# Nature40/pyradiotracking

Measured on AMD Instinct MI355X. Metric: IQ MSamples/s analysed (STFT + detect + records), detected-signal parity vs CPU, higher is better.
Workload: dtype f32

## Files before the change

### pyradiotracking_amd/csrc/rt_analyze.hip

```cpp
#include <hip/hip_runtime.h>

#include <algorithm>
#include <cmath>
#include <cstdio>
#include <cstdlib>
#include <cstring>
#include <limits>
#include <new>
#include <string>
#include <type_traits>
#include <vector>

#include "rt_kernels.h"
#include "rt_general.h"
#include "rt_f64.h"
#include "rt_f64_sparse.h"
#include "rt_f64_rescue.h"
#include "rt_cells.h"
#include "rt_present.h"
#include "rt_chain.h"
#include "rt_record_iq.h"
#include "rt_record_stft.h"
#include "rt_record_stft_hop.h"
#include "rt_record_band.h"
// ... 770 lines not shown
        if (!gone && marked) rows[(size_t)kMaskSubList * S + n_sub++] = s;
        if (!gone && !marked) rows[(size_t)kMaskLinList * S + n_lin++] = s;
    }
    *n_lin_present = n_lin;
    *n_sub_present = n_sub;
    *n_absent = n_abs;
}

int upload_mask(rt_handle *h, Slot &sl) {
    const int S = h->cfg.n_streams;
    fill_mask_rows(sl.lc.pc, S, h->lin ? h->h_sub_first.data() : nullptr, sl.h_mask, &sl.n_lin_present, &sl.n_sub_present, &sl.n_absent);
    RT_HIP(h, hipMemcpyAsync(sl.d_mask, sl.h_mask, (size_t)kMaskRows * S * sizeof(int32_t), hipMemcpyHostToDevice, h->s_scan));
    return RT_OK;
}

int upload_chain_rows(rt_handle *h, Slot &sl) {
    const size_t S = (size_t)h->cfg.n_streams;
    std::memcpy(sl.h_chain_rows, sl.lc.cc.src_buf.data(), S * sizeof(int32_t));
    std::memcpy(sl.h_chain_rows + S, sl.lc.cc.src_idx.data(), S * sizeof(int32_t));
    RT_HIP(h, hipMemcpyAsync(sl.d_chain_rows, sl.h_chain_rows, 2 * S * sizeof(int32_t), hipMemcpyHostToDevice, h->s_scan));
    return RT_OK;
}

template <class P>
int enqueue_carry(rt_handle *h, const int32_t *d_absent_list, int n_absent, const P *src, P *dst, int K, int N) {
    const int64_t per = (int64_t)K * N;
    if (n_absent == 0 || per <= 0) return RT_OK;
    const int bps = carry_blocks(per);
    hipLaunchKernelGGL((carry_tails<P>), dim3((unsigned)((int64_t)n_absent * bps)), dim3(kCarryBlock), 0, h->s_scan, d_absent_list, n_absent, bps, src, dst, per);
    RT_HIP(h, hipGetLastError());
    return RT_OK;
}

int enqueue_analysis(rt_handle *h, Slot &sl, int mode, bool *launched = nullptr, bool second_pass_only = false, bool own_means = false) {
    sl.call.rec_cap_used = h->rec_cap;
    const CallCtx &c = sl.call;
    if (mode == RT_MODE_RUNFILTER && c.thr_rerun && !second_pass_only) own_means = true;
    if (launched) *launched = false;
    const MaskedLaunches masked_launches(h, sl);
    const int32_t *const absent = sl.lc.masked ? sl.d_mask + (size_t)kMaskAbsent * h->cfg.n_streams : nullptr;
    if (h->general) {
        int rc = ensure_dense_spec(h);
        if (rc != RT_OK) return rc;
        RT_HIP(h, hipEventRecord(sl.ev_begin, h->s_scan));
        if (launched) *launched = true;
        launch_general(h, c.iq, c.stream_stride, c.n_seg, h->d_spec, h->d_tail[c.tail_write], c.fmt, absent);
        {
            const int64_t cells = (int64_t)h->cfg.n_streams * h->N;
            hipLaunchKernelGGL(row_sums_dense, dim3((unsigned)((cells + 255) / 256)), dim3(256), 0, h->s_scan, h->d_spec, sl.d_psum, h->cfg.n_streams, c.n_seg, h->N);
        }
        RT_HIP(h, hipGetLastError());
        { const int rc2 = enqueue_chain(h, sl, h->s_scan); if (rc2 != RT_OK) return rc2; }
        RT_HIP(h, hipEventRecord(sl.ev_scan, h->s_scan));
        DetectArgs a = make_detect_args(h, sl, c.n_seg, h->N, c.n_seg_last);
        a.prev = call_prev(h, sl);
        a.prev_cols = h->K;
        a.spec = h->d_spec;
        a.psum = sl.d_psum;
        a.chunks = 1;
        launch_detect_dense(h, h->cfg.n_streams, h->s_scan, a);
        RT_HIP(h, hipGetLastError());
        { const int rc2 = enqueue_row_means(h, sl, 1, c.n_seg, h->s_scan); if (rc2 != RT_OK) return rc2; }
        { const int rc2 = enqueue_record_cells(h, sl, h->d_spec, nullptr, 0, h->s_scan); if (rc2 != RT_OK) return rc2; }
        RT_HIP(h, hipEventRecord(sl.ev_done, h->s_scan));
        return RT_OK;
    }
// ... 139 lines not shown
            const double span = (double)(t_max - t_min);
            std::fprintf(stderr, "RT_STAMPS launch span %.1f us, %.2f waves resident per SIMD on average, %.1f %% of a wave's life inside the step loop; ",
                         span / 100.0, resident / span / 1024.0, 100.0 * sum[13] / resident);
            const double steps = sum[11];
            double tot = 0;
            for (int k = 0; k <= 10; ++k) tot += sum[k];
            std::fprintf(stderr, "RT_STAMPS nperseg %d: %.0f waves, %.1f steps per wave, %.0f cycles per step, in-kernel clock %.0f MHz:", h->N, waves,
                         steps / waves, tot / steps, sum[13] > 0 ? sum[12] / sum[13] * 100.0 : 0.0);
            for (int k = 0; k <= 10; ++k) std::fprintf(stderr, " [%d] %.0f", k, sum[k] / steps);
            std::fprintf(stderr, "\n");
        }
#endif
    }
    RT_HIP(h, hipGetLastError());
    const bool two_scans = !dense && (mode == RT_MODE_RUNFILTER || mode == RT_MODE_PREFILTER);
    { const int rc = enqueue_chain(h, sl, two_scans ? s2 : h->s_scan); if (rc != RT_OK) return rc; }
    RT_HIP(h, hipEventRecord(sl.ev_scan, two_scans ? s2 : h->s_scan));
    if (sd != (two_scans ? s2 : h->s_scan)) RT_HIP(h, hipStreamWaitEvent(sd, sl.ev_scan, 0));
    DetectArgs a = make_detect_args(h, sl, c.n_seg, h->N, c.n_seg_last);
    a.prev = call_prev(h, sl);
    a.prev_cols = h->K;
    a.chunks = sp.blocks_per_stream;
    a.spec = h->d_spec;
    a.filtered = (mode == RT_MODE_PREFILTER || mode == RT_MODE_RUNFILTER) ? 1 : 0;
    if (mode == RT_MODE_RUNFILTER) {
        a.seg_total = sp.seg_count + S;
        a.host_seg_total = sl.h_seg_total;
    }
    if (dense) {
        launch_detect_dense(h, S, sd, a);
    } else {
        if (a.work_list) {
            hipLaunchKernelGGL(detect_group, dim3((S + 3) / 4), dim3(256), h->lds_small, sd, a);
            hipLaunchKernelGGL(detect_bucket_listed, dim3(std::min(S * kQuarters, 1024)), dim3(256), h->lds_small, sd, a);
        } else {
            const int waves = S * kBuckets;
            hipLaunchKernelGGL(detect_bucket<false>, dim3((waves + 3) / 4), dim3(256), h->lds_small, sd, a);
        }
        hipLaunchKernelGGL(detect_bucket<true>, dim3(S), dim3(256), h->lds_large, sd, a);
        if (sl.d_cells) hipLaunchKernelGGL(cells_keep_counts, dim3((S * kBuckets + 255) / 256), dim3(256), 0, sd, sl.d_hot_count, sl.d_hot_kept, S * kBuckets);
        hipLaunchKernelGGL(finalize_records, dim3(S), dim3(256), 0, sd, a);
    }
    RT_HIP(h, hipGetLastError());
    { const int rc = enqueue_row_means(h, sl, sp.blocks_per_stream, c.n_seg, sd); if (rc != RT_OK) return rc; }
    { const int rc = enqueue_record_cells(h, sl, dense ? h->d_spec : nullptr, nullptr, 0, sd); if (rc != RT_OK) return rc; }
    RT_HIP(h, hipEventRecord(sl.ev_done, sd));
    return RT_OK;
}

int enqueue_partial_dense(rt_handle *h, Slot &sl, int n_list, unsigned long long records_so_far) {
    const CallCtx &c = sl.call;
    const int n_part = std::min(h->cfg.n_streams, kMaxPartial);
    if (!h->d_spec_part) {
        const size_t bytes = (size_t)n_part * (size_t)h->max_seg * (size_t)h->N * sizeof(float);
        hipError_t e = hipMalloc(&h->d_spec_part, bytes ? bytes : 4);
        if (e != hipSuccess) {
            h->d_spec_part = nullptr;
            h->err = "dense spectrogram scratch for the partial re-run (" + std::to_string(bytes) + " bytes): " + hipGetErrorString(e);
            return RT_E_NOMEM;
        }
    }
    StftParams sp = make_stft_params(h, sl, c.iq, c.stream_stride, c.n_seg, c.tail_write);
    sp.n_streams = n_list;
    sp.stream_list = sl.h_list;
    sp.spec = h->d_spec_part;
    *sl.h_total = records_so_far;
    RT_HIP(h, hipMemcpyAsync(sl.d_counters, sl.h_total, sizeof(unsigned long long), hipMemcpyHostToDevice, h->s_scan));
    launch_scan<1>(h, sp, n_list * sp.blocks_per_stream, c.fmt);
    RT_HIP(h, hipGetLastError());
    { const int rc = enqueue_chain(h, sl, h->s_scan); if (rc != RT_OK) return rc; }
    DetectArgs a = make_detect_args(h, sl, c.n_seg, h->N, c.n_seg_last);
    a.prev = call_prev(h, sl);
// ... 1567 lines not shown
        if (cfg->mode == RT_MODE_PREFILTER && !h->ap.lv.prefilter_ok) {
            delete h;
            return fail_create(RT_E_UNSUPPORTED, "RT_MODE_PREFILTER needs signal_min_duration >= 2 * segs_per_chunk STFT hops");
        }
        h->two_level = scan_wave64(R3) && !h->ap.lv.prefilter_ok && !RT_DIAG_ENV("RT_EXP_ONE_LEVEL");
        if (h->two_level) {
            h->max_chunks += h->max_chunks / 4 + 2;
            max_blocks_per_stream = (h->max_chunks + h->GPW - 1) / h->GPW;
            h->max_blocks = max_blocks_per_stream;
        }
        h->run_cells = (int)std::max<long long>(1, std::min<long long>(r_min, 1 << 20));
        const bool fits = !general && !big && h->LG >= 4 && std::min<long long>(h->run_cells, (long long)h->max_seg + 1) <= kPlanMaxRun && h->max_seg >= 2;
        if (cfg->mode == RT_MODE_RUNFILTER && !fits) {
            delete h;
            return fail_create(RT_E_UNSUPPORTED, "RT_MODE_RUNFILTER: the minimum plateau length (in STFT hops) is beyond the planner's counters");
        }
        h->ap.lv.runfilter_ok = fits && (cfg->mode == RT_MODE_RUNFILTER || cfg->mode == RT_MODE_AUTO);
        if (h->ap.lv.runfilter_ok && cfg->mode == RT_MODE_AUTO) {
            const size_t per_slot = (size_t)cfg->n_streams * std::max(h->max_seg, 1) * (size_t)(h->LG * 4 + 4) + (size_t)cfg->n_streams * h->N * 4 * (size_t)(h->max_blocks + 2);
            size_t free_b = 0, total_b = 0;
            if (hipMemGetInfo(&free_b, &total_b) != hipSuccess || (size_t)kSlots * per_slot > free_b / (h->ap.lv.prefilter_ok ? 8 : 2)) h->ap.lv.runfilter_ok = false;
        }
    }
    if (!general && ((long long)h->N << key_tbits(std::max(h->max_seg, 2))) > 0x100000000ll) {
        delete h;
        return fail_create(RT_E_UNSUPPORTED, "max_samples too large for 32-bit cell keys");
    }
    h->hot_cap = general ? 64
                 : cfg->hot_capacity > 0
                     ? cfg->hot_capacity
                     : std::min(8192, std::max(kSmallBucket, next_pow2(std::max(h->max_seg, 1)) * std::max(1, h->N / 1024)));
    h->lds_dense = rec_lds_bytes(h->rec_cap);
    {
        h->cand_cap = (h->N / kBuckets <= 32) ? 32 : kCandCapMax;
        const size_t tail = (((size_t)(h->N / kBuckets) * 4 + 15) & ~(size_t)15) + sizeof(rt_record) * h->cand_cap;
        h->lds_large = (size_t)next_pow2(std::max(h->hot_cap, 64)) * 8 + tail;
        h->lds_small = 4 * ((size_t)kSmallBucket * 8 + tail);
    }
    if (h->lds_large + 8 * 1024 > 160 * 1024) {
        delete h;
        return fail_create(RT_E_INVALID, "hot_capacity does not fit the 160 KiB LDS of a CU");
    }
    {
        int fbits = 0;
        while ((1 << fbits) < h->N) ++fbits;
        const bool can = !general && h->N <= kGroupBins && fbits + key_tbits(std::max(h->max_seg, 1)) + 10 <= 32;
        const bool want = (cfg->flags & RT_FLAG_GROUP_DETECT) ? true : (cfg->flags & RT_FLAG_NO_GROUP_DETECT) ? false
                          : cfg->n_streams >= 1024 || (g_creating_lane && (cfg->flags & kFlagLaneOfLargeBatch));
        h->group_detect = can && want;
        h->group_forced = (cfg->flags & RT_FLAG_GROUP_DETECT) != 0;
    }

    auto fail = [&](int code, const std::string &msg) {
        std::string m = msg;
        rt_destroy(h);
        return fail_create(code, m);
    };
#define RT_CREATE_HIP(expr)                                                                  \
    do {                                                                                     \
        hipError_t e2_ = (expr);                                                             \
        if (e2_ != hipSuccess) return fail(RT_E_HIP, std::string(#expr) + ": " + hipGetErrorString(e2_)); \
    } while (0)

    if (cfg->hip_stream) {
        h->s_scan = static_cast<hipStream_t>(cfg->hip_stream);
        h->s_detect = h->s_scan;
    } else {
        RT_CREATE_HIP(hipStreamCreateWithFlags(&h->s_scan, hipStreamNonBlocking));
        h->own_scan_stream = true;
        bool second = R3 <= 2 && !big && !g_creating_lane;
// ... 117 lines not shown
        RT_CREATE_HIP(hipHostMalloc(&sl.h_dc_flag, (size_t)S * sizeof(int32_t)));
        std::memset(sl.h_dc_flag, 0, (size_t)S * sizeof(int32_t));
        RT_CREATE_HIP(hipHostMalloc(&sl.h_list, (size_t)kMaxPartial * sizeof(int32_t)));
        RT_CREATE_HIP(hipHostMalloc(&sl.h_total, sizeof(unsigned long long)));
        if (cfg->flags & RT_FLAG_ROW_MEANS) RT_CREATE_HIP(hipMalloc(&sl.d_row_means, (size_t)S * N * sizeof(float)));
        if (cfg->flags & RT_FLAG_RECORD_CELLS) {
            sl.cell_cap = std::max<int64_t>(64, std::min<int64_t>(kInitialPoolCells, 16 * sl.pool_cap));
            RT_CREATE_HIP(hipMalloc(&sl.d_cells, (size_t)sl.cell_cap * sizeof(float)));
            RT_DEVICE_ZEROS(RT_CREATE_HIP, sl.d_hot_kept, (size_t)S * kBuckets * sizeof(uint32_t));
            RT_CREATE_HIP(hipMalloc(&sl.d_stream_cells, (size_t)S * sizeof(long long)));
            RT_CREATE_HIP(hipMalloc(&sl.d_stream_base, (size_t)S * sizeof(long long)));
            RT_CREATE_HIP(hipHostMalloc(&sl.h_cells_info, 2 * sizeof(unsigned long long)));
            sl.h_cells_info[0] = sl.h_cells_info[1] = 0ull;
        }
        RT_CREATE_HIP(hipEventCreate(&sl.ev_begin));
        RT_CREATE_HIP(hipEventCreateWithFlags(&sl.ev_first, hipEventDisableTiming));
        RT_CREATE_HIP(hipEventCreate(&sl.ev_scan));
        RT_CREATE_HIP(hipEventCreate(&sl.ev_done));
    }

    if (big) {
#define RT_WG_SET(B_, M_, U_, W_) RT_CREATE_HIP(hipFuncSetAttribute(reinterpret_cast<const void *>(stft_wg<B_, M_, U_, W_>), hipFuncAttributeMaxDynamicSharedMemorySize, (int)wg_lds_bytes(B_)))
#define RT_WG_SET4(B_, M_) RT_WG_SET(B_, M_, false, false); RT_WG_SET(B_, M_, false, true); RT_WG_SET(B_, M_, true, false); RT_WG_SET(B_, M_, true, true); \
    RT_WG_SET(B_, M_ | kModeI16, false, false); RT_WG_SET(B_, M_ | kModeI16, false, true); \
    RT_WG_SET(B_, M_ | kModeI8, false, false); RT_WG_SET(B_, M_ | kModeI8, false, true)
        RT_WG_SET4(256, 0); RT_WG_SET4(256, 1); RT_WG_SET4(256, 2);
        RT_WG_SET4(512, 0); RT_WG_SET4(512, 1); RT_WG_SET4(512, 2);
#undef RT_WG_SET4
#undef RT_WG_SET
    }
    RT_CREATE_HIP(hipFuncSetAttribute(reinterpret_cast<const void *>(detect_bucket<true>),
                                      hipFuncAttributeMaxDynamicSharedMemorySize, (int)h->lds_large));
    RT_CREATE_HIP(hipFuncSetAttribute(reinterpret_cast<const void *>(detect_bucket<false>),
                                      hipFuncAttributeMaxDynamicSharedMemorySize, (int)h->lds_small));
    RT_CREATE_HIP(hipFuncSetAttribute(reinterpret_cast<const void *>(detect_group), hipFuncAttributeMaxDynamicSharedMemorySize, (int)h->lds_small));
    RT_CREATE_HIP(hipFuncSetAttribute(reinterpret_cast<const void *>(detect_bucket_listed), hipFuncAttributeMaxDynamicSharedMemorySize, (int)h->lds_small));
    RT_CREATE_HIP(hipFuncSetAttribute(reinterpret_cast<const void *>(detect_dense<false>), hipFuncAttributeMaxDynamicSharedMemorySize,
                                      (int)rec_lds_bytes(kDenseLdsRecords)));
#undef RT_CREATE_HIP
    *out = h;
    return RT_OK;
}

int rt_reset(rt_handle *h) {
    if (!h) return RT_E_INVALID;
    forget_row_means(h);
    for (rt_handle *k : h->kids) rt_reset(k);
    h->ledger.forget_all();
    return RT_OK;
}

int rt_reset_stream(rt_handle *h, int32_t stream) {
    if (!h) return RT_E_INVALID;
    if (stream < 0 || stream >= h->cfg.n_streams) {
        h->err = "stream index out of range";
        return RT_E_INVALID;
    }
    if (!h->kids.empty()) {
        for (size_t k = 0; k < h->kids.size(); ++k)
            if (stream < h->kid_base[k + 1]) return rt_reset_stream(h->kids[k], stream - h->kid_base[k]);
        return RT_E_INVALID;
    }
    h->ledger.reset_stream(stream);
    return RT_OK;
}

static int refuse_on_f64(rt_handle *h, const char *what, const char *twin) {
    h->err = std::string(what) + " on a float64 handle (rt_create_f64): " + (twin ? std::string("use ") + twin : std::string("not available"));
    return RT_E_INVALID;
// ... 2038 lines not shown
```

### pyradiotracking_amd/csrc/rt_core.h

```cpp
#ifndef RT_CORE_H
#define RT_CORE_H

#include <math.h>
#include <stdint.h>

#include <algorithm>
#include <cmath>
#include <initializer_list>
#include <type_traits>
#include <utility>
#include <vector>

#if defined(__HIP__)
#define RT_HD __host__ __device__ __forceinline__
#else
#define RT_HD inline
#endif

namespace rt {

struct cf {
    float x, y;
};
struct cd {
// ... 163 lines not shown


inline int tail_cols(int nperseg, double fs, double max_d) {
    const double hop = seg_time(1, nperseg, fs) - seg_time(0, nperseg, fs);
    const double k = std::floor(max_d / hop) + 2.0;
    const int K = (int)std::min(k, 1.0e6);
    return K < 1 ? 1 : K;
}

inline long long min_run_cells(int N, double fs, double min_d) {
    const double hop = seg_time(1, N, fs) - seg_time(0, N, fs);
    const double cells = min_d * (1.0 - 1e-9) / hop;
    return (long long)std::ceil(std::min(cells, 1.0e9)) - 1;
}

inline int next_pow2(int v) {
    int p = 1;
    while (p < v) p <<= 1;
    return p;
}

inline int key_tbits(int n_seg) {
    int t = 1;
    while ((1ll << t) < (long long)n_seg) ++t;
    return t;
}

constexpr int kBuckets = 16;
constexpr int kSmallBucket = 1024;
constexpr int kQuarters = 4;
constexpr int kCandCapMax = 64;
constexpr int kGroupCells = 896;
constexpr int kGroupBins = 256;

constexpr int kGeneralMaxN = 16384;
struct ScanFamily {
    int R3 = 0, QS = 0, big = 0;
    bool general = false, bluestein = false;
    bool supported = false;
};
inline ScanFamily scan_family(int nperseg) {
    ScanFamily f;
    for (int r : {1, 2, 4, 8, 16})
        if (nperseg == 256 * r) f.R3 = r;
    for (int q : {2, 4, 8})
        if (nperseg == 16 * q) {
            f.R3 = 1;
            f.QS = q;
        }
    if (nperseg == 8192 || nperseg == 16384) {
        f.R3 = 1;
        f.big = nperseg / 32;
    }
    f.supported = true;
    if (!f.R3) {
        const int n = nperseg;
        const bool pow2 = n > 0 && (n & (n - 1)) == 0;
        f.supported = !(n < 8 || (pow2 && n > kGeneralMaxN) || (!pow2 && n > kGeneralMaxN / 2));
        f.general = true;
        f.bluestein = !pow2;
        f.R3 = 1;
    }
    return f;
}

inline int choose_chunk(int nperseg, int R3, int QS, int block, double fs, double min_duration_s, int segs_per_chunk, int n_streams, int n_seg) {
// ... 515 lines not shown
```

### pyradiotracking_amd/csrc/rt_hostcheck.cpp

```cpp
#include <algorithm>
#include <cstdint>
#include <cstring>
#include <numeric>
#include <vector>

#include "../../include/rt_analyze.h"
#include "rt_core.h"
#include "rt_input_stats.h"
#include "rt_ledger.h"
#include "rt_record_stft_book.h"
#include "rt_tables.h"

using namespace rt;

extern "C" {

long long hc_timedelta_us(double seconds) { return (long long)timedelta_us(seconds); }

int hc_probe_stride(int nperseg, double fs, double min_d) { return probe_stride(nperseg, fs, min_d); }

double hc_seg_time(int k, int nperseg, double fs) { return seg_time(k, nperseg, fs); }

int hc_tail_cols(int nperseg, double fs, double max_d) { return tail_cols(nperseg, fs, max_d); }

// ... 193 lines not shown
    return total;
}
}

extern "C" {
long long hc_record_cells(const float *spec, int n_bins, const float *last, int n_seg_last, const rt_record *rec, int n, long long *offsets,
                          float *cells, long long cap) {
    return record_cells_host(spec, n_bins, last, n_seg_last, rec, n, offsets, cells, cap);
}
long long hc_record_cells_f64(const double *spec, int n_bins, const double *last, int n_seg_last, const rt_record_f64 *rec, int n,
                              long long *offsets, double *cells, long long cap) {
    return record_cells_host(spec, n_bins, last, n_seg_last, rec, n, offsets, cells, cap);
}
}

extern "C" {

void hc_scan_family(int nperseg, int *out) {
    const ScanFamily f = scan_family(nperseg);
    const int v[6] = {f.R3, f.QS, f.big, f.general, f.bluestein, f.supported};
    std::memcpy(out, v, sizeof v);
}
int hc_choose_chunk(int nperseg, int block, double fs, double min_d, int segs_per_chunk, int n_streams, int n_seg) {
    const ScanFamily f = scan_family(nperseg);
    return choose_chunk(nperseg, f.R3, f.QS, block, fs, min_d, segs_per_chunk, n_streams, n_seg);
}
long long hc_min_run_cells(int nperseg, double fs, double min_d) { return min_run_cells(nperseg, fs, min_d); }
int hc_key_tbits(int n_seg) { return key_tbits(n_seg); }
void hc_detect_order_constants(int *out) {
    const int v[6] = {kBuckets, kSmallBucket, kGroupCells, kGroupBins, kQuarters, kCandCapMax};
    std::memcpy(out, v, sizeof v);
}
int hc_next_pow2(int v) { return next_pow2(v); }

void hc_scan_twiddles(int N, int R3, int QS, int big, int wave64, cf *tw1, cf *tw2, int *n) {
    const ScanTwiddles t = scan_twiddles(N, R3, QS, big, wave64 != 0);
    n[0] = (int)t.tw1.size();
    n[1] = (int)t.tw2.size();
    if (tw1) std::memcpy(tw1, t.tw1.data(), t.tw1.size() * sizeof(cf));
    if (tw2) std::memcpy(tw2, t.tw2.data(), t.tw2.size() * sizeof(cf));
}
void hc_scaled_window(const float *window, int N, float scale, float *ws) {
    const std::vector<float> v = scaled_window(window, N, scale);
    std::memcpy(ws, v.data(), v.size() * sizeof(float));
}
void hc_window_thread_order(const float *ws, int N, int big, float *out) {
    const std::vector<float> v = window_thread_order(std::vector<float>(ws, ws + N), N, big);
    std::memcpy(out, v.data(), v.size() * sizeof(float));
}
void hc_window_lane_order(const float *ws, int N, int LG, int wave64, float *out) {
    const std::vector<float> v = window_lane_order(std::vector<float>(ws, ws + N), N, LG, wave64 != 0);
    std::memcpy(out, v.data(), v.size() * sizeof(float));
}
int hc_fit_cosine_window(const float *ws, int N, double *wr, double *wi) {
    const CosineFit f = fit_cosine_window(std::vector<float>(ws, ws + N), N);
    std::memcpy(wr, f.wr, sizeof f.wr);
    std::memcpy(wi, f.wi, sizeof f.wi);
    return f.cosine_sum ? 1 : 0;
}
void hc_transform_twiddles_f32(int M, cf *out) {
    const std::vector<cf> v = transform_twiddles<cf, double>(M);
    std::memcpy(out, v.data(), v.size() * sizeof(cf));
}
void hc_transform_twiddles_f64(int M, cd *out) {
    const std::vector<cd> v = transform_twiddles<cd, long double>(M);
    std::memcpy(out, v.data(), v.size() * sizeof(cd));
// ... 481 lines not shown
```

### pyradiotracking_amd/csrc/rt_kernels.h

```cpp
#ifndef RT_KERNELS_H
#define RT_KERNELS_H

#include <hip/hip_runtime.h>
#include <stdint.h>

#include <type_traits>

#include "../../include/rt_analyze.h"
#include "rt_diag.h"
#include "rt_core.h"
#include "rt_fft.h"

namespace rt {

constexpr int kBlock = 256;
constexpr int kRowF2 = 18;

struct StftParams {
    const void *iq;
    int64_t stream_stride;
    int32_t n_streams;
    int32_t n_seg;
    int32_t segs_per_chunk;
    int32_t chunks;
// ... 397 lines not shown
            const u4 v = __builtin_nontemporal_load(reinterpret_cast<const u4 *>(p + 4 * h));
            dst[(4 * h) * QS + m] = iq_i16{v.x};
            dst[(4 * h + 1) * QS + m] = iq_i16{v.y};
            dst[(4 * h + 2) * QS + m] = iq_i16{v.z};
            dst[(4 * h + 3) * QS + m] = iq_i16{v.w};
        }
    }
}

#ifndef RT_ONE_WAVE_MAX_R3
#define RT_ONE_WAVE_MAX_R3 0
#endif
#ifndef RT_NO_PERSIST
#define RT_NO_PERSIST 0
#endif
__device__ __forceinline__ int g_of(unsigned tid, int lg) { return (int)tid / lg; }
__host__ __device__ constexpr bool scan_persistent(int R3, int mode) { return mode != 5 && mode != 7 && !RT_NO_PERSIST && R3 >= 4; }
__host__ __device__ constexpr int scan_block(int R3) { return R3 <= RT_ONE_WAVE_MAX_R3 ? 64 : kBlock; }

#ifndef RT_EXP_DMA1024
#define RT_EXP_DMA1024 0
#endif
constexpr int kModeI16 = 16, kModeI8 = 32;
__host__ __device__ constexpr int scan_fmt(int modef, bool u8) { return (modef & kModeI8) ? kFmtI8 : (modef & kModeI16) ? kFmtI16 : u8 ? kFmtU8 : kFmtC64; }
__host__ __device__ constexpr bool scan_dma(int r3, int fmt, int qs) { return RT_EXP_DMA1024 && r3 == 4 && fmt == kFmtC64 && qs == 0; }
__device__ void raw_buffer_load_lds_fwd(rsrc_t rsrc, __attribute__((address_space(3))) void *lds, int size, int voffset, int soffset, int offset, int aux)
    __asm("llvm.amdgcn.raw.buffer.load.lds");
#ifndef RT_WG4_MAX_R3
#define RT_WG4_MAX_R3 0
#endif
#ifndef RT_PK_R3_MASK
#define RT_PK_R3_MASK (1 | 4)
#endif
#ifndef RT_EXP_U8_PK
#define RT_EXP_U8_PK 0
#endif
__host__ __device__ constexpr int scan_wgs_per_cu(int r3, int fmt, int qs) {
    return scan_dma(r3, fmt, qs) ? 2 : (r3 <= RT_WG4_MAX_R3 || (fmt == kFmtU8 && r3 == 1 && !RT_EXP_U8_PK)) ? 4 : 3;
}
template <int R3, int MODEF, bool U8 = false, bool LIN = false, int QS = 0>
__global__ __launch_bounds__(scan_block(R3), scan_wgs_per_cu(R3, scan_fmt(MODEF, U8), QS))
 void stft_scan(const StftParams p) {
    constexpr int MODE = MODEF & (kModeI16 - 1);
    constexpr int FMT = scan_fmt(MODEF, U8);
    using raw_t = typename raw_of<FMT>::type;
    static_assert(QS == 0 || (R3 == 1 && (QS == 2 || QS == 4 || QS == 8)), "QS: lane groups of 2 / 4 / 8 lanes, R3 = 1");
    constexpr int N = QS ? 16 * QS : 256 * R3;
    constexpr int LG = QS ? QS : 16 * R3;
    constexpr int PER = QS ? 16 / QS : 1;
    constexpr int BLK = scan_block(R3);
    constexpr int GPW = BLK / LG;
    constexpr int G = 16 / R3;
    constexpr int ROW = (QS == 2) ? 16 : kRowF2;
    constexpr int GPAD = (U8 && QS == 8) ? 0 : QS;

    constexpr bool W_IN_LDS = (R3 <= 8);
    constexpr bool T1_IN_LDS = (R3 <= 4) && !scan_dma(R3, FMT, QS);
    constexpr bool T1_FACTORED = !T1_IN_LDS;
    constexpr bool DMA = scan_dma(R3, FMT, QS);
    constexpr int kStage = (R3 <= RT_WG4_MAX_R3 || (U8 && R3 == 1 && !RT_EXP_U8_PK)) ? 32 : (R3 == 8) ? 96 : DMA ? 64 : kStageCap;
    constexpr size_t kXchB = sizeof(cf) * (BLK * ROW + GPW * GPAD);
    constexpr size_t kRedB = (LG > 64) ? sizeof(cf) * (BLK / 64) + 16 + sizeof(uint32_t) * (BLK / 64) : 0;
    constexpr size_t kWB = W_IN_LDS ? sizeof(float4) * 4 * LG : 0;
    constexpr size_t kT1fB = T1_FACTORED ? sizeof(float4) * 2 * LG : 0;
    constexpr size_t kT1B = T1_IN_LDS ? sizeof(float4) * 8 * LG : 0;
    constexpr size_t kT2B = (R3 > 1) ? sizeof(float4) * 8 * R3 : 0;
    constexpr size_t kStageB = (MODE == 0 || MODE == 5 || MODE == 7) ? sizeof(uint2) * (BLK / 64) * kStage : 0;
    constexpr bool THR_LDS = (MODE == 6) && R3 <= 4;
    constexpr size_t kThrB = THR_LDS ? sizeof(float) * N : 0;
    constexpr bool BITS_LDS = (MODE == 6) && R3 <= 2 && (QS == 0 || QS >= 4);
    constexpr size_t kBitsB = BITS_LDS ? sizeof(uint16_t) * 4 * BLK : 0;
    constexpr size_t kDmaB = DMA ? sizeof(cf) * N * (BLK / 64) : 0;
    __shared__ __attribute__((aligned(16))) unsigned char lds_block[kXchB + kRedB + kWB + kT1fB + kT1B + kT2B + kStageB + kThrB + kBitsB + kDmaB];
    cf *const landing = reinterpret_cast<cf *>(lds_block + kXchB + kRedB + kWB + kT1fB + kT1B + kT2B + kStageB + kThrB + kBitsB) + (DMA ? __builtin_amdgcn_readfirstlane((int)(threadIdx.x >> 6)) * N : 0);
    uint16_t *const bits_lds = reinterpret_cast<uint16_t *>(lds_block + kXchB + kRedB + kWB + kT1fB + kT1B + kT2B + kStageB + kThrB) + (BITS_LDS ? g_of(threadIdx.x, LG) * 4 * LG : 0);
    float4 *const thr_lds = reinterpret_cast<float4 *>(lds_block + kXchB + kRedB + kWB + kT1fB + kT1B + kT2B + kStageB);
    cf *const xch = reinterpret_cast<cf *>(lds_block);
    cf *const red = reinterpret_cast<cf *>(lds_block + kXchB);
    uint32_t *const tail_any = reinterpret_cast<uint32_t *>(lds_block + kXchB + sizeof(cf) * (BLK / 64));
    uint32_t *const red_const = tail_any + 4;

    const int tid = threadIdx.x;
    const int g = tid / LG;
    const int lt = tid % LG;
    const int T = p.n_seg;
    const int L = p.segs_per_chunk;

    constexpr bool PK = ((RT_PK_R3_MASK & R3) != 0) && (!U8 || (RT_EXP_U8_PK && R3 == 1));
    using C = typename std::conditional<PK, cfv, cf>::type;
    C *gx = reinterpret_cast<C *>(xch + g * (LG * ROW + GPAD));

    float4 *const w_lds = reinterpret_cast<float4 *>(lds_block + kXchB + kRedB);
    float4 *const t1f_lds = reinterpret_cast<float4 *>(lds_block + kXchB + kRedB + kWB);
    float4 *const t1_lds = reinterpret_cast<float4 *>(lds_block + kXchB + kRedB + kWB + kT1fB);
    float4 *const t2_lds = reinterpret_cast<float4 *>(lds_block + kXchB + kRedB + kWB + kT1fB + kT1B);
    if constexpr (W_IN_LDS) {
        for (int idx = tid; idx < 4 * LG; idx += BLK) {
            const int mm = idx / LG, l = idx % LG;
            if constexpr (QS) {
                auto smp = [&](int r) { return p.window[PER * l + r / QS + 16 * (r % QS)]; };
                w_lds[idx] = make_float4(smp(4 * mm), smp(4 * mm + 1), smp(4 * mm + 2), smp(4 * mm + 3));
            } else {
                w_lds[idx] = make_float4(p.window[l + LG * (4 * mm)], p.window[l + LG * (4 * mm + 1)],
                                         p.window[l + LG * (4 * mm + 2)], p.window[l + LG * (4 * mm + 3)]);
            }
        }
    }
    if constexpr (T1_IN_LDS) {
        for (int idx = tid; idx < 8 * LG; idx += BLK) {
            const int kk = idx / LG, l = idx % LG;
            const cf a = p.tw1[l * 16 + 2 * kk], b = p.tw1[l * 16 + 2 * kk + 1];
            t1_lds[idx] = make_float4(a.x, a.y, b.x, b.y);
        }
    }
    if constexpr (T1_FACTORED) {
        for (int l = tid; l < LG; l += BLK) {
            const cf w1 = p.tw1[l * 16 + 1], w2 = p.tw1[l * 16 + 2], w4 = p.tw1[l * 16 + 4], w8 = p.tw1[l * 16 + 8];
            t1f_lds[l] = make_float4(w1.x, w1.y, w2.x, w2.y);
            t1f_lds[LG + l] = make_float4(w4.x, w4.y, w8.x, w8.y);
        }
    }
// ... 1840 lines not shown
                keys[i] = e.x;
                vals[i] = __uint_as_float(e.y);
            } else {
                keys[i] = 0xFFFFFFFFu;
                vals[i] = 0.f;
            }
        }
        __syncthreads();
        for (int k = 2; k <= n2; k <<= 1) {
            for (int j = k >> 1; j > 0; j >>= 1) {
                for (int t = tid; t < (n2 >> 1); t += 256) {
                    const int i = ((t & ~(j - 1)) << 1) | (t & (j - 1));
                    const int ixj = i | j;
                    const bool up = ((i & k) == 0);
                    const uint32_t ki = keys[i], kj = keys[ixj];
                    if ((ki > kj) == up) {
                        keys[i] = kj;
                        keys[ixj] = ki;
                        const float tv = vals[i];
                        vals[i] = vals[ixj];
                        vals[ixj] = tv;
                    }
                }
                __syncthreads();
            }
        }
        if (wave != 0) return;
    }

    detect_runs(a, dp, s, n, keys, vals, cand, lane, [&](int bin) -> float { return avg[bin / kBuckets]; });
}

template <bool LARGE>
__global__ __launch_bounds__(256) void detect_bucket(const DetectArgs a) {
    extern __shared__ __attribute__((aligned(16))) unsigned char dyn_smem[];
    const int wave = __builtin_amdgcn_readfirstlane((int)(threadIdx.x >> 6));
    const int lane = (int)__builtin_amdgcn_mbcnt_hi(~0u, __builtin_amdgcn_mbcnt_lo(~0u, 0u));
    if constexpr (!LARGE) {
        detect_bucket_one<false>(a, (int)blockIdx.x * 4 + wave, wave, lane, dyn_smem);
    } else {
        if ((int)blockIdx.x >= a.n_streams || a.large_any[blockIdx.x] == 0u) return;
        for (int b = 0; b < kBuckets; ++b) {
            detect_bucket_one<true>(a, (int)blockIdx.x * kBuckets + b, wave, lane, dyn_smem);
            __syncthreads();
        }
    }
}


template <int M>
__device__ __forceinline__ void sort_group_packed(const uint2 *hot_s, const int hot_cap, const uint32_t (&ends)[kBuckets], const int n, const int lane,
                                                  uint32_t *keys, float *vals) {
    constexpr int kIdxBits = 10;
    uint32_t k[M];
#pragma unroll
    for (int m = 0; m < M; ++m) {
        const uint32_t i = (uint32_t)(m * 64 + lane);
        uint32_t b = 0u, st = 0u;
#pragma unroll
        for (int j = 0; j < kBuckets; ++j) {
            const bool ge = i >= ends[j];
            b += ge ? 1u : 0u;
            st = ge ? ends[j] : st;
        }
        uint32_t word = 0xFFFFFFFFu;
        if (i < (uint32_t)n) {
            const uint2 e = hot_s[(int64_t)b * hot_cap + (i - st)];
            word = (e.x << kIdxBits) | i;
            keys[i] = e.y;
        }
        k[m] = word;
    }
    wave_sync();
    wave_bitonic_sort_u32<M>(k, lane);
    float v[M];
#pragma unroll
    for (int m = 0; m < M; ++m) v[m] = (m * 64 + lane < n) ? __uint_as_float(keys[k[m] & ((1u << kIdxBits) - 1u)]) : 0.f;
// ... 50 lines not shown
    const int nbins_b = F / kBuckets;
    const size_t wave_bytes = (size_t)kSmallBucket * 8 + (((size_t)nbins_b * 4 + 15) & ~(size_t)15) + sizeof(rt_record) * a.cand_cap;
    unsigned char *base = dyn_smem + (size_t)wave * wave_bytes;
    uint32_t *keys = reinterpret_cast<uint32_t *>(base);
    float *vals = reinterpret_cast<float *>(keys + kGroupCells);
    float *avg = vals + kGroupCells;
    rt_record *cand = reinterpret_cast<rt_record *>(base + (size_t)kSmallBucket * 8 + (((size_t)nbins_b * 4 + 15) & ~(size_t)15));
    const DetectParams dp = stream_params(a, s);
    const uint2 *hot_s = a.hot + (int64_t)s * kBuckets * a.hot_cap;
    int n2 = 64;
    while (n2 < n) n2 <<= 1;
    switch (n2) {
        case 64: sort_group_packed<1>(hot_s, a.hot_cap, ends, n, lane, keys, vals); break;
        case 128: sort_group_packed<2>(hot_s, a.hot_cap, ends, n, lane, keys, vals); break;
        case 256: sort_group_packed<4>(hot_s, a.hot_cap, ends, n, lane, keys, vals); break;
        case 512: sort_group_packed<8>(hot_s, a.hot_cap, ends, n, lane, keys, vals); break;
        default: sort_group_packed<16>(hot_s, a.hot_cap, ends, n, lane, keys, vals); break;
    }
    wave_sync();
    if (RT_DETECT_ABLATE == 3) return;
    for (int base_i = 0; base_i < n; base_i += 64) {
        const int i = base_i + lane;
        if (i < n) {
            const int bin = (int)(keys[i] >> a.tbits);
            if (i == 0 || (int)(keys[i - 1] >> a.tbits) != bin)
                avg[bin] = (float)row_sum_from_partials(a.psum + (int64_t)s * a.chunks * F + bin, a.chunks, F) / (float)T;
        }
    }
    wave_sync();
    if (RT_DETECT_ABLATE == 7) return;
    detect_runs(a, dp, s, n, keys, vals, cand, lane, [&](int bin) -> float { return avg[bin]; });
}

__global__ __launch_bounds__(256) void detect_bucket_listed(const DetectArgs a) {
    extern __shared__ __attribute__((aligned(16))) unsigned char dyn_smem[];
    const int wave = __builtin_amdgcn_readfirstlane((int)(threadIdx.x >> 6));
    const int lane = (int)__builtin_amdgcn_mbcnt_hi(~0u, __builtin_amdgcn_mbcnt_lo(~0u, 0u));
    const int n_work = __builtin_amdgcn_readfirstlane(*a.work_count);
    for (int w = (int)blockIdx.x; w < n_work; w += (int)gridDim.x) {
        const int e = __builtin_amdgcn_readfirstlane(a.work_list[w]);
        detect_bucket_one<false>(a, (e / kQuarters) * kBuckets + (e % kQuarters) * (kBuckets / kQuarters) + wave, wave, lane, dyn_smem);
        wave_sync();
    }
}

constexpr int kFinalTile = 256;
constexpr int kTicketShift = 40;
__global__ __launch_bounds__(256) void finalize_records(const DetectArgs a) {
    __shared__ rt_record t_rec[kFinalTile];
    __shared__ long long t_ts[kFinalTile], t_dur[kFinalTile];
    __shared__ long long sh_base;
    __shared__ int sh_fit;
    const int s = a.stream_list ? a.stream_list[blockIdx.x] : (int)blockIdx.x;
    const int tid = threadIdx.x;
    int n = a.raw_count[s];
    uint32_t hot_sum = 0u;
    if (!a.stream_list && tid < 64) {
        uint32_t c = 0u;
        if (tid < kBuckets) {
            c = a.hot_count[s * kBuckets + tid];
            if (c) a.hot_count_rw[s * kBuckets + tid] = 0u;
        }
        const auto addu = [](uint32_t x, uint32_t y) { return x + y; };
        hot_sum = butterfly_step<1>(butterfly_step<2>(butterfly_step<4>(butterfly_step<8>(c, addu), addu), addu), addu);
    }
    const int wanted = n;
    if (n > a.rec_cap) n = a.rec_cap;
    if (n < 0) n = 0;
    __syncthreads();
    if (tid == 0) {
        if (wanted) a.raw_count[s] = 0;
        if (wanted > a.rec_cap) {
            atomicOr(&a.counters[2], kFlagRecOverflow);
            atomicMax(&a.counters[4], (unsigned long long)wanted);
// ... 234 lines not shown
```

Baseline: 766,100.

## Launch detect kernels as single-wave blocks and grid-stride large bucket streams

The small-bucket detect kernels now run one 64-thread wave per block with a quarter of the LDS, where before four waves shared a 256-thread block. The aim is better CU packing and no waiting on the slowest wave in a block. The large-bucket kernel now uses a capped grid that finds streams needing work with a wave ballot and strides over them, instead of launching one block per stream that often exits at once. A compile-time flag also turns off the packed FFT path for C64 R3=1 QS=0, which adds a separate codegen change to the STFT.

After: 764,300. About the same (-0.2%).

```diff
diff --git a/pyradiotracking_amd/csrc/rt_analyze.hip b/pyradiotracking_amd/csrc/rt_analyze.hip
--- a/pyradiotracking_amd/csrc/rt_analyze.hip
+++ b/pyradiotracking_amd/csrc/rt_analyze.hip
@@ -826,6 +826,8 @@
     return RT_OK;
 }
 
+inline int large_grid(int S) { return std::min(S, std::max(16, std::min(256, S / 4))); }
+
 int enqueue_analysis(rt_handle *h, Slot &sl, int mode, bool *launched = nullptr, bool second_pass_only = false, bool own_means = false) {
     sl.call.rec_cap_used = h->rec_cap;
     const CallCtx &c = sl.call;
@@ -1031,12 +1033,11 @@
     } else {
         if (a.work_list) {
             hipLaunchKernelGGL(detect_group, dim3((S + 3) / 4), dim3(256), h->lds_small, sd, a);
-            hipLaunchKernelGGL(detect_bucket_listed, dim3(std::min(S * kQuarters, 1024)), dim3(256), h->lds_small, sd, a);
+            hipLaunchKernelGGL(detect_bucket_listed, dim3(std::min(S * kBuckets, 4096)), dim3(64), h->lds_small / 4, sd, a);
         } else {
-            const int waves = S * kBuckets;
-            hipLaunchKernelGGL(detect_bucket<false>, dim3((waves + 3) / 4), dim3(256), h->lds_small, sd, a);
-        }
-        hipLaunchKernelGGL(detect_bucket<true>, dim3(S), dim3(256), h->lds_large, sd, a);
+            hipLaunchKernelGGL(detect_bucket<false>, dim3(S * kBuckets), dim3(64), h->lds_small / 4, sd, a);
+        }
+        hipLaunchKernelGGL(detect_bucket<true>, dim3(large_grid(S)), dim3(256), h->lds_large, sd, a);
         if (sl.d_cells) hipLaunchKernelGGL(cells_keep_counts, dim3((S * kBuckets + 255) / 256), dim3(256), 0, sd, sl.d_hot_count, sl.d_hot_kept, S * kBuckets);
         hipLaunchKernelGGL(finalize_records, dim3(S), dim3(256), 0, sd, a);
     }
@@ -2670,10 +2671,10 @@
                      : std::min(8192, std::max(kSmallBucket, next_pow2(std::max(h->max_seg, 1)) * std::max(1, h->N / 1024)));
     h->lds_dense = rec_lds_bytes(h->rec_cap);
     {
-        h->cand_cap = (h->N / kBuckets <= 32) ? 32 : kCandCapMax;
-        const size_t tail = (((size_t)(h->N / kBuckets) * 4 + 15) & ~(size_t)15) + sizeof(rt_record) * h->cand_cap;
+        h->cand_cap = detect_cand_cap(h->N);
+        const size_t tail = detect_lds_tail(h->N, sizeof(rt_record));
         h->lds_large = (size_t)next_pow2(std::max(h->hot_cap, 64)) * 8 + tail;
-        h->lds_small = 4 * ((size_t)kSmallBucket * 8 + tail);
+        h->lds_small = 4 * detect_wave_lds(h->N, sizeof(rt_record));
     }
     if (h->lds_large + 8 * 1024 > 160 * 1024) {
         delete h;
@@ -2857,9 +2858,9 @@
     RT_CREATE_HIP(hipFuncSetAttribute(reinterpret_cast<const void *>(detect_bucket<true>),
                                       hipFuncAttributeMaxDynamicSharedMemorySize, (int)h->lds_large));
     RT_CREATE_HIP(hipFuncSetAttribute(reinterpret_cast<const void *>(detect_bucket<false>),
-                                      hipFuncAttributeMaxDynamicSharedMemorySize, (int)h->lds_small));
+                                      hipFuncAttributeMaxDynamicSharedMemorySize, (int)(h->lds_small / 4)));
     RT_CREATE_HIP(hipFuncSetAttribute(reinterpret_cast<const void *>(detect_group), hipFuncAttributeMaxDynamicSharedMemorySize, (int)h->lds_small));
-    RT_CREATE_HIP(hipFuncSetAttribute(reinterpret_cast<const void *>(detect_bucket_listed), hipFuncAttributeMaxDynamicSharedMemorySize, (int)h->lds_small));
+    RT_CREATE_HIP(hipFuncSetAttribute(reinterpret_cast<const void *>(detect_bucket_listed), hipFuncAttributeMaxDynamicSharedMemorySize, (int)(h->lds_small / 4)));
     RT_CREATE_HIP(hipFuncSetAttribute(reinterpret_cast<const void *>(detect_dense<false>), hipFuncAttributeMaxDynamicSharedMemorySize,
                                       (int)rec_lds_bytes(kDenseLdsRecords)));
 #undef RT_CREATE_HIP
diff --git a/pyradiotracking_amd/csrc/rt_core.h b/pyradiotracking_amd/csrc/rt_core.h
--- a/pyradiotracking_amd/csrc/rt_core.h
+++ b/pyradiotracking_amd/csrc/rt_core.h
@@ -219,6 +219,9 @@
 constexpr int kCandCapMax = 64;
 constexpr int kGroupCells = 896;
 constexpr int kGroupBins = 256;
+inline int detect_cand_cap(int N) { return (N / kBuckets <= 32) ? 32 : kCandCapMax; }
+inline size_t detect_lds_tail(int N, size_t record_bytes) { return (((size_t)(N / kBuckets) * 4 + 15) & ~(size_t)15) + record_bytes * (size_t)detect_cand_cap(N); }
+inline size_t detect_wave_lds(int N, size_t record_bytes) { return (size_t)kSmallBucket * 8 + detect_lds_tail(N, record_bytes); }
 
 constexpr int kGeneralMaxN = 16384;
 struct ScanFamily {
diff --git a/pyradiotracking_amd/csrc/rt_hostcheck.cpp b/pyradiotracking_amd/csrc/rt_hostcheck.cpp
--- a/pyradiotracking_amd/csrc/rt_hostcheck.cpp
+++ b/pyradiotracking_amd/csrc/rt_hostcheck.cpp
@@ -249,6 +249,7 @@
     std::memcpy(out, v, sizeof v);
 }
 int hc_next_pow2(int v) { return next_pow2(v); }
+long long hc_detect_wave_lds(int nperseg) { return (long long)detect_wave_lds(nperseg, sizeof(rt_record)); }
 
 void hc_scan_twiddles(int N, int R3, int QS, int big, int wave64, cf *tw1, cf *tw2, int *n) {
     const ScanTwiddles t = scan_twiddles(N, R3, QS, big, wave64 != 0);
diff --git a/pyradiotracking_amd/csrc/rt_kernels.h b/pyradiotracking_amd/csrc/rt_kernels.h
--- a/pyradiotracking_amd/csrc/rt_kernels.h
+++ b/pyradiotracking_amd/csrc/rt_kernels.h
@@ -453,6 +453,9 @@
 #ifndef RT_PK_R3_MASK
 #define RT_PK_R3_MASK (1 | 4)
 #endif
+#ifndef RT_SCALAR_C64_256
+#define RT_SCALAR_C64_256 1
+#endif
 #ifndef RT_EXP_U8_PK
 #define RT_EXP_U8_PK 0
 #endif
@@ -507,7 +510,7 @@
     const int T = p.n_seg;
     const int L = p.segs_per_chunk;
 
-    constexpr bool PK = ((RT_PK_R3_MASK & R3) != 0) && (!U8 || (RT_EXP_U8_PK && R3 == 1));
+    constexpr bool PK = ((RT_PK_R3_MASK & R3) != 0) && !(RT_SCALAR_C64_256 && FMT == kFmtC64 && R3 == 1 && QS == 0) && (!U8 || (RT_EXP_U8_PK && R3 == 1));
     using C = typename std::conditional<PK, cfv, cf>::type;
     C *gx = reinterpret_cast<C *>(xch + g * (LG * ROW + GPAD));
 
@@ -2414,17 +2417,25 @@
 }
 
 template <bool LARGE>
-__global__ __launch_bounds__(256) void detect_bucket(const DetectArgs a) {
+__global__ __launch_bounds__(LARGE ? 256 : 64) void detect_bucket(const DetectArgs a) {
     extern __shared__ __attribute__((aligned(16))) unsigned char dyn_smem[];
-    const int wave = __builtin_amdgcn_readfirstlane((int)(threadIdx.x >> 6));
     const int lane = (int)__builtin_amdgcn_mbcnt_hi(~0u, __builtin_amdgcn_mbcnt_lo(~0u, 0u));
     if constexpr (!LARGE) {
-        detect_bucket_one<false>(a, (int)blockIdx.x * 4 + wave, wave, lane, dyn_smem);
+        detect_bucket_one<false>(a, (int)blockIdx.x, 0, lane, dyn_smem);
     } else {
-        if ((int)blockIdx.x >= a.n_streams || a.large_any[blockIdx.x] == 0u) return;
-        for (int b = 0; b < kBuckets; ++b) {
-            detect_bucket_one<true>(a, (int)blockIdx.x * kBuckets + b, wave, lane, dyn_smem);
-            __syncthreads();
+        const int wave = __builtin_amdgcn_readfirstlane((int)(threadIdx.x >> 6));
+        for (int j0 = 0; (int)blockIdx.x + j0 * (int)gridDim.x < a.n_streams; j0 += 64) {
+            const int sj = (int)blockIdx.x + (j0 + lane) * (int)gridDim.x;
+            unsigned long long todo = __builtin_amdgcn_ballot_w64(sj < a.n_streams && a.large_any[sj < a.n_streams ? sj : 0] != 0u);
+            while (todo) {
+                const int j = __builtin_ctzll(todo);
+                todo &= todo - 1ull;
+                const int s = (int)blockIdx.x + (j0 + j) * (int)gridDim.x;
+                for (int b = 0; b < kBuckets; ++b) {
+                    detect_bucket_one<true>(a, s * kBuckets + b, wave, lane, dyn_smem);
+                    __syncthreads();
+                }
+            }
         }
     }
 }
@@ -2541,14 +2552,14 @@
     detect_runs(a, dp, s, n, keys, vals, cand, lane, [&](int bin) -> float { return avg[bin]; });
 }
 
-__global__ __launch_bounds__(256) void detect_bucket_listed(const DetectArgs a) {
+__global__ __launch_bounds__(64, 4) void detect_bucket_listed(const DetectArgs a) {
     extern __shared__ __attribute__((aligned(16))) unsigned char dyn_smem[];
-    const int wave = __builtin_amdgcn_readfirstlane((int)(threadIdx.x >> 6));
+    constexpr int QB = kBuckets / kQuarters;
     const int lane = (int)__builtin_amdgcn_mbcnt_hi(~0u, __builtin_amdgcn_mbcnt_lo(~0u, 0u));
-    const int n_work = __builtin_amdgcn_readfirstlane(*a.work_count);
+    const int n_work = __builtin_amdgcn_readfirstlane(*a.work_count) * QB;
     for (int w = (int)blockIdx.x; w < n_work; w += (int)gridDim.x) {
-        const int e = __builtin_amdgcn_readfirstlane(a.work_list[w]);
-        detect_bucket_one<false>(a, (e / kQuarters) * kBuckets + (e % kQuarters) * (kBuckets / kQuarters) + wave, wave, lane, dyn_smem);
+        const int e = __builtin_amdgcn_readfirstlane(a.work_list[w / QB]);
+        detect_bucket_one<false>(a, (e / kQuarters) * kBuckets + (e % kQuarters) * QB + w % QB, 0, lane, dyn_smem);
         wave_sync();
     }
 }
```
